# snap-research/MMVID

Measured on AMD Instinct MI355X. Metric: video-tokens/sec training step, 8-frame 128px text-to-video, higher is better.
Workload: dtype bf16

## Files before the change

### mmvid_amd/csrc/common.h

```cpp
#pragma once
#include <hip/hip_runtime.h>
#include <stdint.h>
#include <stdio.h>
#include <stdlib.h>
#include <string.h>

typedef uint16_t bf16_t;
typedef __attribute__((ext_vector_type(8))) __bf16 bf16x8_t;
typedef __attribute__((ext_vector_type(8))) _Float16 f16x8_t;
typedef __attribute__((ext_vector_type(4))) float f32x4;
typedef __attribute__((ext_vector_type(16))) float f32x16;

#define MMVID_OK 0
#define MMVID_ERR_ARG 1
#define MMVID_ERR_HIP 2

extern "C" const char* mmvid_last_error();
void mmvid_set_error(const char* fmt, ...);

#define MMVID_REQUIRE(cond, ...)          \
    do {                                  \
        if (!(cond)) {                    \
            mmvid_set_error(__VA_ARGS__); \
            return MMVID_ERR_ARG;         \
        }                                 \
    } while (0)

#define MMVID_LAUNCH_CHECK(name)                                               \
    do {                                                                       \
        hipError_t e__ = hipGetLastError();                                    \
        if (e__ != hipSuccess) {                                               \
            mmvid_set_error("%s: launch failed: %s", name, hipGetErrorString(e__)); \
            return MMVID_ERR_HIP;                                              \
        }                                                                      \
    } while (0)

typedef __attribute__((ext_vector_type(2))) float f32x2;
typedef __attribute__((ext_vector_type(2))) __bf16 bf16x2_t;
__device__ __forceinline__ float bf2f(bf16_t v) { return __uint_as_float(((uint32_t)v) << 16); }
__device__ __forceinline__ uint32_t pack_bf2(float lo, float hi) {
    const f32x2 v = {lo, hi};
    return __builtin_bit_cast(uint32_t, __builtin_convertvector(v, bf16x2_t));
}
__device__ __forceinline__ bf16_t f2bf(float f) { return (bf16_t)(pack_bf2(f, f) & 0xffffu); }
__device__ __forceinline__ float bf_lo(uint32_t w) { return __uint_as_float(w << 16); }
__device__ __forceinline__ float bf_hi(uint32_t w) { return __uint_as_float(w & 0xffff0000u); }

__device__ __forceinline__ float sigmoidf_(float x) { return 1.0f / (1.0f + __expf(-x)); }

__device__ __forceinline__ float wave_sum(float v) {
#pragma unroll
    for (int o = 32; o > 0; o >>= 1) v += __shfl_xor(v, o, 64);
    return v;
}
__device__ __forceinline__ float wave_max(float v) {
#pragma unroll
    for (int o = 32; o > 0; o >>= 1) v = fmaxf(v, __shfl_xor(v, o, 64));
    return v;
}

template <int CTRL>
__device__ __forceinline__ float dpp_mov(float v) {
    return __builtin_bit_cast(float, __builtin_amdgcn_update_dpp(0, __builtin_bit_cast(int, v), CTRL, 0xf, 0xf, true));
}
__device__ __forceinline__ float wave_sum_fast(float v) {
    v += dpp_mov<0xB1>(v);
    v += dpp_mov<0x4E>(v);
    v += dpp_mov<0x141>(v);
    v += dpp_mov<0x140>(v);
    const uint32_t u = __float_as_uint(v);
    const auto r = __builtin_amdgcn_permlane16_swap(u, u, false, false);
    v = __uint_as_float(r[0]) + __uint_as_float(r[1]);
    const uint32_t w = __float_as_uint(v);
    const auto q = __builtin_amdgcn_permlane32_swap(w, w, false, false);
    return __uint_as_float(q[0]) + __uint_as_float(q[1]);
}
__device__ __forceinline__ float wave_max_fast(float v) {
    v = fmaxf(v, dpp_mov<0xB1>(v));
    v = fmaxf(v, dpp_mov<0x4E>(v));
    v = fmaxf(v, dpp_mov<0x141>(v));
    v = fmaxf(v, dpp_mov<0x140>(v));
    const uint32_t u = __float_as_uint(v);
    const auto r = __builtin_amdgcn_permlane16_swap(u, u, false, false);
    v = fmaxf(__uint_as_float(r[0]), __uint_as_float(r[1]));
    const uint32_t w = __float_as_uint(v);
    const auto q = __builtin_amdgcn_permlane32_swap(w, w, false, false);
    return fmaxf(__uint_as_float(q[0]), __uint_as_float(q[1]));
}

__device__ __forceinline__ void mfma_settle(f32x16& acc) { asm volatile("s_nop 15" : "+v"(acc)); }
__device__ __forceinline__ void mfma_settle(f32x4& acc) { asm volatile("s_nop 15" : "+v"(acc)); }

static inline int cdiv(long a, long b) { return (int)((a + b - 1) / b); }
static inline float* gn_stats_partials(float* area, int N, int C) { return area + (long)N * C * 2; }
enum { MMVID_OPT_GRAPHS = 0, MMVID_OPT_DETERMINISTIC = 1, MMVID_OPT_COUNT = 2 };
int mmvid_option(int which);
int mmvid_slab_reduce(const float* slab, int nslabs, int N, float* out, hipStream_t stream);
unsigned long long* mmvid_fault_counters_dev();
```

### mmvid_amd/csrc/norm.hip

```cpp
#include "../../include/mmvid_hip.h"
#include "common.h"
#include <type_traits>

namespace {

constexpr int LN_MAXV = 4;

__global__ __launch_bounds__(256) void layernorm_fwd_kernel(const float* __restrict__ x, long ldx, long rows, int E,
                                                            const float* __restrict__ w,
                                                            const float* __restrict__ b, float eps,
                                                            bf16_t* __restrict__ y_bf16, float* __restrict__ y_f32,
                                                            long ldy, float* __restrict__ mean_out,
                                                            float* __restrict__ rstd_out) {
    const long half = (rows + 1) >> 1;
    const long r0 = (long)blockIdx.x * 4 + (threadIdx.x >> 6);
    if (r0 >= half) return;
    const long rr[2] = {r0, r0 + half};
    const bool live1 = rr[1] < rows;
    const int lane = threadIdx.x & 63;
    const int nv = E >> 2;
    float4 v[2][LN_MAXV];
    float s[2] = {0.f, 0.f};
#pragma unroll
    for (int k = 0; k < 2; ++k) {
        const float4* xr = reinterpret_cast<const float4*>(x + (k == 0 || live1 ? rr[k] : rr[0]) * ldx);
#pragma unroll
        for (int i = 0; i < LN_MAXV; ++i) {
            const int c = lane + 64 * i;
            v[k][i] = c < nv ? xr[c] : make_float4(0, 0, 0, 0);
        }
    }
#pragma unroll
    for (int k = 0; k < 2; ++k)
#pragma unroll
        for (int i = 0; i < LN_MAXV; ++i) s[k] += (v[k][i].x + v[k][i].y) + (v[k][i].z + v[k][i].w);
    const float mean[2] = {wave_sum_fast(s[0]) / (float)E, wave_sum_fast(s[1]) / (float)E};
    float q[2] = {0.f, 0.f};
#pragma unroll
    for (int k = 0; k < 2; ++k)
#pragma unroll
        for (int i = 0; i < LN_MAXV; ++i) {
            const int c = lane + 64 * i;
            if (c < nv) {
                const float a = v[k][i].x - mean[k], b2 = v[k][i].y - mean[k], c2 = v[k][i].z - mean[k], d = v[k][i].w - mean[k];
                q[k] += (a * a + b2 * b2) + (c2 * c2 + d * d);
            }
        }
    const float rstd[2] = {rsqrtf(wave_sum_fast(q[0]) / (float)E + eps), rsqrtf(wave_sum_fast(q[1]) / (float)E + eps)};
#pragma unroll
    for (int k = 0; k < 2; ++k) {
        if (k == 1 && !live1) break;
        const long r = rr[k];
        if (lane == 0) {
            if (mean_out) mean_out[r] = mean[k];
            if (rstd_out) rstd_out[r] = rstd[k];
        }
#pragma unroll
        for (int i = 0; i < LN_MAXV; ++i) {
            const int c = lane + 64 * i;
            if (c < nv) {
                const float4 w4 = reinterpret_cast<const float4*>(w)[c];
                const float4 b4 = reinterpret_cast<const float4*>(b)[c];
                float4 o;
                o.x = (v[k][i].x - mean[k]) * rstd[k] * w4.x + b4.x;
                o.y = (v[k][i].y - mean[k]) * rstd[k] * w4.y + b4.y;
                o.z = (v[k][i].z - mean[k]) * rstd[k] * w4.z + b4.z;
                o.w = (v[k][i].w - mean[k]) * rstd[k] * w4.w + b4.w;
                if (y_f32) reinterpret_cast<float4*>(y_f32 + r * ldy)[c] = o;
                if (y_bf16) reinterpret_cast<uint2*>(y_bf16 + r * ldy)[c] = make_uint2(pack_bf2(o.x, o.y), pack_bf2(o.z, o.w));
            }
        }
    }
}

template <typename DY>
__global__ __launch_bounds__(256) void layernorm_bwd_kernel(const DY* __restrict__ dy, long lddy,
                                                            const float* __restrict__ x, long ldx,
                                                            const float* __restrict__ mean,
                                                            const float* __restrict__ rstd,
                                                            const float* __restrict__ w, long rows, int E,
                                                            float* __restrict__ dx, long lddx, int add,
                                                            bf16_t* __restrict__ dx_bf16,
                                                            float* __restrict__ dw, float* __restrict__ db,
                                                            float* __restrict__ dx_colsum, float* __restrict__ partial) {
    __shared__ float red[2][4][LN_MAXV * 64 * 4];
    const int lane = threadIdx.x & 63, wave = threadIdx.x >> 6;
    const int nv = E >> 2;
    float4 pw[LN_MAXV], pb[LN_MAXV], pc[LN_MAXV], w4[LN_MAXV];
#pragma unroll
    for (int i = 0; i < LN_MAXV; ++i) {
        pw[i] = pb[i] = pc[i] = make_float4(0, 0, 0, 0);
        const int c = lane + 64 * i;
        w4[i] = (c < nv) ? reinterpret_cast<const float4*>(w)[c] : make_float4(0, 0, 0, 0);
    }
    for (long r = (long)blockIdx.x * 4 + wave; r < rows; r += (long)gridDim.x * 4) {
        const float mu = mean[r], rs = rstd[r];
        float4 g[LN_MAXV], xh[LN_MAXV], prev[LN_MAXV];
        float s1 = 0.f, s2 = 0.f;
#pragma unroll
        for (int i = 0; i < LN_MAXV; ++i) {
            const int c = lane + 64 * i;
            if (c < nv) {
                prev[i] = add ? reinterpret_cast<const float4*>(dx + r * lddx)[c] : make_float4(0.f, 0.f, 0.f, 0.f);
                float4 d4;
                if constexpr (sizeof(DY) == 4) {
                    d4 = reinterpret_cast<const float4*>(dy + r * lddy)[c];
                } else {
                    const uint2 u = reinterpret_cast<const uint2*>(dy + r * lddy)[c];
                    d4 = make_float4(bf_lo(u.x), bf_hi(u.x), bf_lo(u.y), bf_hi(u.y));
                }
                const float4 x4 = reinterpret_cast<const float4*>(x + r * ldx)[c];
                xh[i] = make_float4((x4.x - mu) * rs, (x4.y - mu) * rs, (x4.z - mu) * rs, (x4.w - mu) * rs);
                g[i] = make_float4(d4.x * w4[i].x, d4.y * w4[i].y, d4.z * w4[i].z, d4.w * w4[i].w);
                s1 += (g[i].x + g[i].y) + (g[i].z + g[i].w);
                s2 += (g[i].x * xh[i].x + g[i].y * xh[i].y) + (g[i].z * xh[i].z + g[i].w * xh[i].w);
                pw[i].x += d4.x * xh[i].x, pw[i].y += d4.y * xh[i].y, pw[i].z += d4.z * xh[i].z, pw[i].w += d4.w * xh[i].w;
                pb[i].x += d4.x, pb[i].y += d4.y, pb[i].z += d4.z, pb[i].w += d4.w;
            }
        }
        const float m1 = wave_sum_fast(s1) / (float)E, m2 = wave_sum_fast(s2) / (float)E;
#pragma unroll
        for (int i = 0; i < LN_MAXV; ++i) {
            const int c = lane + 64 * i;
            if (c < nv) {
                float4 o;
                o.x = rs * (g[i].x - m1 - xh[i].x * m2);
                o.y = rs * (g[i].y - m1 - xh[i].y * m2);
                o.z = rs * (g[i].z - m1 - xh[i].z * m2);
                o.w = rs * (g[i].w - m1 - xh[i].w * m2);
                float4* d = reinterpret_cast<float4*>(dx + r * lddx) + c;
                o.x += prev[i].x, o.y += prev[i].y, o.z += prev[i].z, o.w += prev[i].w;
                *d = o;
                pc[i].x += o.x, pc[i].y += o.y, pc[i].z += o.z, pc[i].w += o.w;
                if (dx_bf16)
                    reinterpret_cast<uint2*>(dx_bf16 + r * lddx)[c] = make_uint2(pack_bf2(o.x, o.y), pack_bf2(o.z, o.w));
            }
        }
    }
// ... 395 lines not shown
        }
        const long at = ((long)n * hw + p) * C + c0 + cc * 8;
        if (y_bf16)
            *reinterpret_cast<uint4*>(y_bf16 + at) = make_uint4(pack_bf2(o[0], o[1]), pack_bf2(o[2], o[3]), pack_bf2(o[4], o[5]), pack_bf2(o[6], o[7]));
        if (y_f32) {
            float4* d = reinterpret_cast<float4*>(y_f32 + at);
            d[0] = make_float4(o[0], o[1], o[2], o[3]);
            d[1] = make_float4(o[4], o[5], o[6], o[7]);
        }
    }
}

__global__ __launch_bounds__(256) void groupnorm_finalize_f64_kernel(const float* __restrict__ partial, int nblk, int N, int C,
                                                                     double cnt, float eps, float* __restrict__ mr) {
    const int item = blockIdx.x * 4 + (threadIdx.x >> 6);
    if (item >= N * 32) return;
    const int lane = threadIdx.x & 63;
    const int n = item >> 5, grp = item & 31;
    double sm = 0.0, sq = 0.0;
    for (int k = lane; k < nblk; k += 64) {
        const float2 v = *reinterpret_cast<const float2*>(partial + (((long)n * nblk + k) * 32 + grp) * 2);
        sm += (double)v.x, sq += (double)v.y;
    }
    for (int o = 32; o > 0; o >>= 1) sm += __shfl_xor(sm, o, 64), sq += __shfl_xor(sq, o, 64);
    const double mu = sm / cnt;
    double var = sq / cnt - mu * mu;
    var = var < 0.0 ? 0.0 : var;
    const double rstd = 1.0 / sqrt(var + (double)eps);
    const int cpg = C >> 5;
    if (lane < cpg) *reinterpret_cast<float2*>(mr + ((long)n * C + grp * cpg + lane) * 2) = make_float2((float)mu, (float)rstd);
}

template <bool F16>
__global__ __launch_bounds__(256) void groupnorm_apply_split_kernel(const float* __restrict__ x, long hw, int C,
                                                                    const float* __restrict__ mr, const float* __restrict__ w,
                                                                    const float* __restrict__ b, int swish,
                                                                    bf16_t* __restrict__ planes, long total_chunks) {
    const long t = (long)blockIdx.x * 256 + threadIdx.x;
    if (t >= total_chunks) return;
    const int cchunks = C >> 3;
    const int cc = (int)(t % cchunks);
    const long pix = t / cchunks;
    const int n = (int)(pix / hw);
    float f[8], wv[8], bv[8];
    load8<float>(x + pix * C + cc * 8, f);
    load8<float>(w + cc * 8, wv);
    load8<float>(b + cc * 8, bv);
    const float4* q = reinterpret_cast<const float4*>(mr + ((long)n * C + cc * 8) * 2);
    const float4 q0 = q[0], q1 = q[1], q2 = q[2], q3 = q[3];
    const float mu[8] = {q0.x, q0.z, q1.x, q1.z, q2.x, q2.z, q3.x, q3.z};
    const float rs[8] = {q0.y, q0.w, q1.y, q1.w, q2.y, q2.w, q3.y, q3.w};
    uint32_t h[4], l[4];
    float o[8];
#pragma unroll
    for (int e = 0; e < 8; ++e) {
        float v = ((f[e] - mu[e]) * rs[e]) * wv[e] + bv[e];
        if (swish) v = v * (1.0f / (1.0f + expf(-v)));
        o[e] = v;
    }
    if constexpr (F16) {
#pragma unroll
        for (int e = 0; e < 4; ++e) {
            typedef __attribute__((ext_vector_type(2))) _Float16 h2_t;
            const h2_t p2 = {(_Float16)o[2 * e], (_Float16)o[2 * e + 1]};
            h[e] = __builtin_bit_cast(uint32_t, p2);
        }
        *reinterpret_cast<uint4*>(planes + t * 8) = make_uint4(h[0], h[1], h[2], h[3]);
        return;
    }
#pragma unroll
    for (int e = 0; e < 4; ++e) {
        h[e] = pack_bf2(o[2 * e], o[2 * e + 1]);
        l[e] = pack_bf2(o[2 * e] - bf_lo(h[e]), o[2 * e + 1] - bf_hi(h[e]));
    }
    *reinterpret_cast<uint4*>(planes + t * 8) = make_uint4(h[0], h[1], h[2], h[3]);
    *reinterpret_cast<uint4*>(planes + (total_chunks + t) * 8) = make_uint4(l[0], l[1], l[2], l[3]);
}

}

extern "C" int mmvid_layernorm_fwd(const float* x, int64_t ldx, int64_t rows, int E, const float* w, const float* b,
                                   float eps, void* y_bf16, float* y_f32, int64_t ldy, float* mean, float* rstd,
                                   void* stream) {
    MMVID_REQUIRE(x && w && b && (y_bf16 || y_f32), "layernorm_fwd: null pointer");
    MMVID_REQUIRE(E % 4 == 0 && E <= 64 * 4 * LN_MAXV && ldx % 4 == 0 && ldy % 4 == 0,
                  "layernorm_fwd: E=%d must be a multiple of 4 and <= %d; row strides multiples of 4", E,
                  64 * 4 * LN_MAXV);
    if (rows == 0) return MMVID_OK;
    hipLaunchKernelGGL(layernorm_fwd_kernel, dim3(cdiv((rows + 1) / 2, 4)), dim3(256), 0, (hipStream_t)stream, x, (long)ldx,
                       (long)rows, E, w, b, eps, (bf16_t*)y_bf16, y_f32, (long)ldy, mean, rstd);
    MMVID_LAUNCH_CHECK("layernorm_fwd");
    return MMVID_OK;
}

extern "C" int mmvid_layernorm_bwd_ws(const float* dy, int64_t lddy, const float* x, int64_t ldx, const float* mean,
                                      const float* rstd, const float* w, int64_t rows, int E, float* dx, int64_t lddx,
                                      int add_into_dx, void* dx_bf16, float* dw, float* db, float* dx_colsum,
                                      float* workspace, int64_t workspace_floats, void* stream);
extern "C" int mmvid_layernorm_bwd_ex(const void* dy, int dy_is_bf16, int64_t lddy, const float* x, int64_t ldx, const float* mean,
                                      const float* rstd, const float* w, int64_t rows, int E, float* dx, int64_t lddx,
                                      int add_into_dx, void* dx_bf16, float* dw, float* db, float* dx_colsum,
                                      float* workspace, int64_t workspace_floats, void* stream);

extern "C" int mmvid_layernorm_bwd(const float* dy, int64_t lddy, const float* x, int64_t ldx, const float* mean,
                                   const float* rstd, const float* w, int64_t rows, int E, float* dx, int64_t lddx,
                                   int add_into_dx, void* dx_bf16, float* dw, float* db, float* dx_colsum,
                                   void* stream) {
    return mmvid_layernorm_bwd_ws(dy, lddy, x, ldx, mean, rstd, w, rows, E, dx, lddx, add_into_dx, dx_bf16, dw, db, dx_colsum,
                                  nullptr, 0, stream);
}

extern "C" int mmvid_layernorm_bwd_ws(const float* dy, int64_t lddy, const float* x, int64_t ldx, const float* mean,
                                      const float* rstd, const float* w, int64_t rows, int E, float* dx, int64_t lddx,
                                      int add_into_dx, void* dx_bf16, float* dw, float* db, float* dx_colsum,
                                      float* workspace, int64_t workspace_floats, void* stream) {
    return mmvid_layernorm_bwd_ex(dy, 0, lddy, x, ldx, mean, rstd, w, rows, E, dx, lddx, add_into_dx, dx_bf16, dw, db, dx_colsum,
                                  workspace, workspace_floats, stream);
}

static int layernorm_bwd_impl(const void* dy, int dy_is_bf16, int64_t lddy, const float* x, int64_t ldx, const float* mean,
                              const float* rstd, const float* w, int64_t rows, int E, float* dx, int64_t lddx, int add_into_dx,
                              void* dx_bf16, float* dw, float* db, float* dx_colsum, float* workspace, int64_t workspace_floats,
                              int* blocks_out, void* stream) {
    MMVID_REQUIRE(dy && x && mean && rstd && w && dx, "layernorm_bwd: null pointer");
    MMVID_REQUIRE(E % 4 == 0 && E <= 64 * 4 * LN_MAXV && lddy % 4 == 0 && ldx % 4 == 0 && lddx % 4 == 0,
                  "layernorm_bwd: bad E/strides");
    if (rows == 0) return MMVID_OK;
    int blocks = cdiv(rows, 4);
    const bool any_red = dw || db || dx_colsum;
    float* partial = nullptr;
    if (workspace && any_red) {
        int cap = (int)(workspace_floats / (3 * (int64_t)E));
        if (cap > 2048) cap = 2048;
        if (cap >= 64) {
            if (blocks > cap) blocks = cap;
            partial = workspace;
        }
    }
    MMVID_REQUIRE(partial || !any_red || !mmvid_option(MMVID_OPT_DETERMINISTIC),
                  "layernorm_bwd: deterministic mode refuses the atomic dw / db / dx_colsum sums: pass a workspace of at least 64 * 3 * E "
                  "floats (mmvid_layernorm_bwd_ws / mmvid_layernorm_bwd_ex / mmvid_layernorm_bwd_partial)");
    if (!partial) {
        if (blocks > 512) blocks = 512;
    }
    float* const a_dw = partial ? (dw ? dw : workspace) : dw;
    float* const a_db = partial ? (db ? db : workspace) : db;
    float* const a_cs = partial ? (dx_colsum ? dx_colsum : nullptr) : dx_colsum;
    if (E == 768 || E == 512) {
#define MMVID_LN_FAST(DYT, NVI)                                                                                                            \
    hipLaunchKernelGGL((layernorm_bwd_fast_kernel<DYT, NVI>), dim3(blocks), dim3(256), 0, (hipStream_t)stream, (const DYT*)dy, (long)lddy, x, \
                       (long)ldx, mean, rstd, w, (long)rows, dx, (long)lddx, add_into_dx, (bf16_t*)dx_bf16, a_dw, a_db, a_cs, partial)
        if (dy_is_bf16) {
            if (E == 768) MMVID_LN_FAST(bf16_t, 3); else MMVID_LN_FAST(bf16_t, 2);
        } else {
            if (E == 768) MMVID_LN_FAST(float, 3); else MMVID_LN_FAST(float, 2);
        }
#undef MMVID_LN_FAST
    } else if (dy_is_bf16)
        hipLaunchKernelGGL(layernorm_bwd_kernel<bf16_t>, dim3(blocks), dim3(256), 0, (hipStream_t)stream, (const bf16_t*)dy, (long)lddy, x,
                           (long)ldx, mean, rstd, w, (long)rows, E, dx, (long)lddx, add_into_dx, (bf16_t*)dx_bf16,
                           partial ? (dw ? dw : workspace) : dw, partial ? (db ? db : workspace) : db,
                           partial ? (dx_colsum ? dx_colsum : nullptr) : dx_colsum, partial);
    else
        hipLaunchKernelGGL(layernorm_bwd_kernel<float>, dim3(blocks), dim3(256), 0, (hipStream_t)stream, (const float*)dy, (long)lddy, x,
                           (long)ldx, mean, rstd, w, (long)rows, E, dx, (long)lddx, add_into_dx, (bf16_t*)dx_bf16,
                           partial ? (dw ? dw : workspace) : dw, partial ? (db ? db : workspace) : db,
                           partial ? (dx_colsum ? dx_colsum : nullptr) : dx_colsum, partial);
    if (blocks_out) {
        MMVID_REQUIRE(partial || !any_red, "layernorm_bwd_partial: needs a workspace of at least 64 * 3 * E floats");
        *blocks_out = blocks;
    } else if (partial) {
        hipLaunchKernelGGL(layernorm_bwd_reduce_kernel, dim3(cdiv(E, 32), 3), dim3(1024), 0, (hipStream_t)stream, partial, blocks, E,
                           dw, db, dx_colsum);
// ... 127 lines not shown
```

### mmvid_amd/csrc/optim.hip

```cpp
#include "../../include/mmvid_hip.h"
#include "common.h"

namespace {

__global__ __launch_bounds__(256) void grad_sqnorm_kernel(const float* __restrict__ g, long n,
                                                          float* __restrict__ out) {
    float a = 0.f;
    const long stride = (long)gridDim.x * 256 * 4;
    for (long i = ((long)blockIdx.x * 256 + threadIdx.x) * 4; i < n; i += stride) {
        if (i + 3 < n) {
            const float4 v = *reinterpret_cast<const float4*>(g + i);
            a += (v.x * v.x + v.y * v.y) + (v.z * v.z + v.w * v.w);
        } else {
            for (long k = i; k < n; ++k) a += g[k] * g[k];
        }
    }
    a = wave_sum(a);
    __shared__ float sh[4];
    if ((threadIdx.x & 63) == 0) sh[threadIdx.x >> 6] = a;
    __syncthreads();
    if (threadIdx.x == 0) unsafeAtomicAdd(out, (sh[0] + sh[1]) + (sh[2] + sh[3]));
}

struct AdamArgs {
    float lr, beta1, beta2, eps, weight_decay, bc1, bc2_sqrt, max_norm, grad_scale;
};
struct LazyRows {
    const unsigned char* flags;
    long lo, hi;
    int rowlen;
};
__device__ __forceinline__ bool lazy_skip(const LazyRows& z, long i) {
    return z.flags && i >= z.lo && i < z.hi && z.flags[(i - z.lo) / z.rowlen] == 0;
}

__global__ __launch_bounds__(256) void adam_kernel(float* __restrict__ p, const float* __restrict__ g,
                                                   float* __restrict__ m, float* __restrict__ v,
                                                   bf16_t* __restrict__ shadow, long n, AdamArgs a,
                                                   const float* __restrict__ sqnorm,
                                                   const float* __restrict__ step_dev,
                                                   const float* __restrict__ lr_dev, LazyRows z) {
    if (lr_dev) a.lr = *lr_dev;
    if (step_dev) {
        const float t = *step_dev;
        a.bc1 = 1.0f - powf(a.beta1, t);
        a.bc2_sqrt = sqrtf(1.0f - powf(a.beta2, t));
    }
    float coef = a.grad_scale;
    if (sqnorm && a.max_norm > 0.f) {
        const float c = a.max_norm / (sqrtf(*sqnorm) * a.grad_scale + 1e-6f);
        coef *= c < 1.f ? c : 1.f;
    }
    const float step = a.lr / a.bc1;
    const long stride = (long)gridDim.x * 256 * 4;
    for (long i = ((long)blockIdx.x * 256 + threadIdx.x) * 4; i < n; i += stride) {
        if (lazy_skip(z, i)) continue;
        if (i + 3 < n) {
            float4 pp = *reinterpret_cast<float4*>(p + i);
            const float4 gg = *reinterpret_cast<const float4*>(g + i);
            float4 mm = *reinterpret_cast<float4*>(m + i), vv = *reinterpret_cast<float4*>(v + i);
            float pe[4] = {pp.x, pp.y, pp.z, pp.w}, ge[4] = {gg.x, gg.y, gg.z, gg.w};
            float me[4] = {mm.x, mm.y, mm.z, mm.w}, ve[4] = {vv.x, vv.y, vv.z, vv.w};
#pragma unroll
            for (int e = 0; e < 4; ++e) {
                float gr = ge[e] * coef + a.weight_decay * pe[e];
                me[e] = a.beta1 * me[e] + (1.f - a.beta1) * gr;
                ve[e] = a.beta2 * ve[e] + (1.f - a.beta2) * gr * gr;
                pe[e] -= step * me[e] / (sqrtf(ve[e]) / a.bc2_sqrt + a.eps);
            }
            *reinterpret_cast<float4*>(p + i) = make_float4(pe[0], pe[1], pe[2], pe[3]);
            *reinterpret_cast<float4*>(m + i) = make_float4(me[0], me[1], me[2], me[3]);
            *reinterpret_cast<float4*>(v + i) = make_float4(ve[0], ve[1], ve[2], ve[3]);
            if (shadow) *reinterpret_cast<uint2*>(shadow + i) = make_uint2(pack_bf2(pe[0], pe[1]), pack_bf2(pe[2], pe[3]));
        } else {
            for (long k = i; k < n; ++k) {
                float gr = g[k] * coef + a.weight_decay * p[k];
                float mk = a.beta1 * m[k] + (1.f - a.beta1) * gr;
                float vk = a.beta2 * v[k] + (1.f - a.beta2) * gr * gr;
                float pk = p[k] - step * mk / (sqrtf(vk) / a.bc2_sqrt + a.eps);
                p[k] = pk, m[k] = mk, v[k] = vk;
                if (shadow) shadow[k] = f2bf(pk);
            }
        }
    }
}

__global__ __launch_bounds__(256) void cast_bf16_kernel(const float* __restrict__ x, bf16_t* __restrict__ y, long n) {
    const long stride = (long)gridDim.x * 256 * 4;
    for (long i = ((long)blockIdx.x * 256 + threadIdx.x) * 4; i < n; i += stride) {
        if (i + 3 < n) {
            const float4 v = *reinterpret_cast<const float4*>(x + i);
            *reinterpret_cast<uint2*>(y + i) = make_uint2(pack_bf2(v.x, v.y), pack_bf2(v.z, v.w));
        } else {
            for (long k = i; k < n; ++k) y[k] = f2bf(x[k]);
        }
    }
}

static int grid_for(long n) {
    long b = (n + 1023) / 1024;
    if (b > 2048) b = 2048;
    if (b < 1) b = 1;
    return (int)b;
}

}

extern "C" int mmvid_grad_sqnorm(const float* g, int64_t n, float* out_accum, void* stream) {
    MMVID_REQUIRE(g && out_accum && n >= 0, "grad_sqnorm: bad arguments");
    MMVID_REQUIRE(((uintptr_t)g & 15) == 0, "grad_sqnorm: buffer must be 16-byte aligned");
    if (n == 0) return MMVID_OK;
    hipLaunchKernelGGL(grad_sqnorm_kernel, dim3(grid_for(n)), dim3(256), 0, (hipStream_t)stream, g, (long)n, out_accum);
    MMVID_LAUNCH_CHECK("grad_sqnorm");
    return MMVID_OK;
}

__global__ __launch_bounds__(256) void grad_sqnorm_partial_kernel(const float* __restrict__ g, long n, float* __restrict__ part,
                                                                  LazyRows z) {
    float a = 0.f;
    const long stride = (long)gridDim.x * 256 * 4;
    for (long i = ((long)blockIdx.x * 256 + threadIdx.x) * 4; i < n; i += stride) {
        if (lazy_skip(z, i)) continue;
        if (i + 3 < n) {
            const float4 v = *reinterpret_cast<const float4*>(g + i);
            a += (v.x * v.x + v.y * v.y) + (v.z * v.z + v.w * v.w);
        } else {
            for (long k = i; k < n; ++k) a += g[k] * g[k];
        }
    }
    a = wave_sum(a);
    __shared__ float sh[4];
    if ((threadIdx.x & 63) == 0) sh[threadIdx.x >> 6] = a;
    __syncthreads();
    if (threadIdx.x == 0) part[blockIdx.x] = (sh[0] + sh[1]) + (sh[2] + sh[3]);
}
__global__ __launch_bounds__(256) void sum_partials_kernel(const float* __restrict__ part, int nb, float* __restrict__ out) {
    __shared__ float sh[256];
    float a = 0.f;
    for (int i = threadIdx.x; i < nb; i += 256) a += part[i];
    sh[threadIdx.x] = a;
    __syncthreads();
    for (int o = 128; o > 0; o >>= 1) {
        if ((int)threadIdx.x < o) sh[threadIdx.x] += sh[threadIdx.x + o];
        __syncthreads();
    }
    if (threadIdx.x == 0) out[0] += sh[0];
}

static int make_lazy(LazyRows& z, const uint8_t* flags, int64_t lo, int64_t rows, int rowlen, int64_t n) {
    z.flags = nullptr, z.lo = z.hi = 0, z.rowlen = 1;
    if (!flags) return MMVID_OK;
    MMVID_REQUIRE(lo >= 0 && rows >= 0 && rowlen > 0 && rowlen % 4 == 0 && lo % 4 == 0 && lo + rows * rowlen <= n,
                  "lazy rows: the table [%lld, +%lld x %d) must lie inside the buffer and be 4-element aligned", (long long)lo,
                  (long long)rows, rowlen);
    z.flags = flags, z.lo = lo, z.hi = lo + rows * rowlen, z.rowlen = rowlen;
    return MMVID_OK;
}

extern "C" int mmvid_grad_sqnorm_det(const float* g, int64_t n, float* partials, float* out_accum, void* stream) {
    return mmvid_grad_sqnorm_rows(g, n, partials, out_accum, nullptr, 0, 0, 0, stream);
}

extern "C" int mmvid_grad_sqnorm_rows(const float* g, int64_t n, float* partials, float* out_accum, const uint8_t* row_flags,
                                      int64_t table_lo, int64_t table_rows, int rowlen, void* stream) {
    MMVID_REQUIRE(g && partials && out_accum && n >= 0, "grad_sqnorm_det: bad arguments");
    MMVID_REQUIRE(((uintptr_t)g & 15) == 0, "grad_sqnorm_det: buffer must be 16-byte aligned");
    if (n == 0) return MMVID_OK;
    LazyRows z;
    if (int rc = make_lazy(z, row_flags, table_lo, table_rows, rowlen, n)) return rc;
    const int nb = grid_for(n);
    hipLaunchKernelGGL(grad_sqnorm_partial_kernel, dim3(nb), dim3(256), 0, (hipStream_t)stream, g, (long)n, partials, z);
    hipLaunchKernelGGL(sum_partials_kernel, dim3(1), dim3(256), 0, (hipStream_t)stream, partials, nb, out_accum);
    MMVID_LAUNCH_CHECK("grad_sqnorm_det");
    return MMVID_OK;
}

extern "C" int mmvid_adam_step_lr(float* p, const float* g, float* m, float* v, void* shadow_bf16, int64_t n, float lr,
                                  const float* lr_dev, float beta1, float beta2, float eps, float weight_decay, int step,
                                  const float* step_dev, float max_norm, const float* sqnorm, float grad_scale, void* stream);

extern "C" int mmvid_adam_step(float* p, const float* g, float* m, float* v, void* shadow_bf16, int64_t n, float lr,
                               float beta1, float beta2, float eps, float weight_decay, int step,
                               const float* step_dev, float max_norm, const float* sqnorm, float grad_scale,
                               void* stream) {
    return mmvid_adam_step_lr(p, g, m, v, shadow_bf16, n, lr, nullptr, beta1, beta2, eps, weight_decay, step, step_dev, max_norm,
                              sqnorm, grad_scale, stream);
}

extern "C" int mmvid_adam_step_lr(float* p, const float* g, float* m, float* v, void* shadow_bf16, int64_t n, float lr,
                                  const float* lr_dev, float beta1, float beta2, float eps, float weight_decay, int step,
                                  const float* step_dev, float max_norm, const float* sqnorm, float grad_scale, void* stream) {
    return mmvid_adam_step_rows(p, g, m, v, shadow_bf16, n, lr, lr_dev, beta1, beta2, eps, weight_decay, step, step_dev, max_norm,
                                sqnorm, grad_scale, nullptr, 0, 0, 0, stream);
}

extern "C" int mmvid_adam_step_rows(float* p, const float* g, float* m, float* v, void* shadow_bf16, int64_t n, float lr,
                                    const float* lr_dev, float beta1, float beta2, float eps, float weight_decay, int step,
                                    const float* step_dev, float max_norm, const float* sqnorm, float grad_scale,
                                    const uint8_t* row_flags, int64_t table_lo, int64_t table_rows, int rowlen, void* stream) {
    MMVID_REQUIRE(p && g && m && v && n >= 0 && (step >= 1 || step_dev), "adam_step: bad arguments");
    MMVID_REQUIRE(!row_flags || weight_decay == 0.f, "adam_step: lazy rows are exact only without weight decay");
    LazyRows z;
    if (int rc = make_lazy(z, row_flags, table_lo, table_rows, rowlen, n)) return rc;
    MMVID_REQUIRE((((uintptr_t)p | (uintptr_t)g | (uintptr_t)m | (uintptr_t)v) & 15) == 0 && ((uintptr_t)shadow_bf16 & 7) == 0,
                  "adam_step: buffers must be 16-byte aligned");
    if (n == 0) return MMVID_OK;
    AdamArgs a;
    a.lr = lr, a.beta1 = beta1, a.beta2 = beta2, a.eps = eps, a.weight_decay = weight_decay;
    a.bc1 = 1.0f - powf(beta1, (float)(step >= 1 ? step : 1));
    a.bc2_sqrt = sqrtf(1.0f - powf(beta2, (float)(step >= 1 ? step : 1)));
    a.max_norm = max_norm, a.grad_scale = grad_scale;
    hipLaunchKernelGGL(adam_kernel, dim3(grid_for(n)), dim3(256), 0, (hipStream_t)stream, p, g, m, v, (bf16_t*)shadow_bf16,
                       (long)n, a, sqnorm, step_dev, lr_dev, z);
    MMVID_LAUNCH_CHECK("adam_step");
    return MMVID_OK;
}

extern "C" int mmvid_cast_f32_to_bf16(const float* x, void* y, int64_t n, void* stream) {
    MMVID_REQUIRE(x && y && n >= 0, "cast_f32_to_bf16: bad arguments");
    MMVID_REQUIRE(((uintptr_t)x & 15) == 0 && ((uintptr_t)y & 7) == 0, "cast_f32_to_bf16: alignment");
    if (n == 0) return MMVID_OK;
    hipLaunchKernelGGL(cast_bf16_kernel, dim3(grid_for(n)), dim3(256), 0, (hipStream_t)stream, x, (bf16_t*)y, (long)n);
    MMVID_LAUNCH_CHECK("cast_f32_to_bf16");
    return MMVID_OK;
}
```

### mmvid_amd/csrc/tower.hip

```cpp
#include "../../include/mmvid_hip.h"
#include "common.h"
#include <vector>

#include "graphs.h"

namespace {

inline int64_t align256(int64_t x) { return (x + 255) & ~(int64_t)255; }
constexpr int kMaxSplitK = 16;
constexpr int kLnBwdBlocks = 512;

struct Dims {
    int B, L, E, H, F, layers;
    int64_t M;
};
Dims dims_of(const mmvid_tower_cfg_t& c) {
    Dims d;
    d.B = c.B, d.L = c.L, d.E = c.E, d.H = c.H, d.F = c.F, d.layers = c.layers;
    d.M = (int64_t)c.B * c.L;
    return d;
}

struct SavedLayer {
    int64_t x_in, x_mid, mean1, rstd1, mean2, rstd2, h1, qkv, o, lse2, h2, pre, act, k_gpj, k_dpre, k_gout, k_dqkv, k_ln1, k_ln2, total;
// ... 53 lines not shown

#define TRY(call)                   \
    do {                            \
        int rc__ = (call);          \
        if (rc__ != 0) return rc__; \
    } while (0)

int check_cfg(const mmvid_tower_cfg_t* c) {
    MMVID_REQUIRE(c, "tower: null config");
    MMVID_REQUIRE(c->B > 0 && c->L > 0 && c->layers > 0, "tower: bad B/L/layers");
    MMVID_REQUIRE(c->E == c->H * 64 && c->E % 8 == 0 && c->F % 8 == 0 && c->E <= 1024,
                  "tower: need E == 64*H <= 1024 and F %% 8 == 0 (E=%d H=%d F=%d)", c->E, c->H, c->F);
    return 0;
}

int linear_fwd(int64_t M, int N, int K, const void* X, const void* W, const float* bias, const float* residual,
               void* save_pre, int act, float* out_f32, void* out_bf16, void* st) {
    return mmvid_gemm_bf16(0, 0, (int)M, N, K, X, K, W, K, 1, 0, 0, 0, 1, 1.0f, bias, residual, N, nullptr, save_pre, N,
                           act, 0, out_f32, out_bf16, N, nullptr, st);
}
int linear_dx(int64_t M, int N, int K, const void* dY, const void* W, const void* dact_pre, float* out_f32,
              void* out_bf16, void* st, float* out_colsum = nullptr, void* det_ws = nullptr, int64_t det_bytes = 0) {
    if (out_colsum && det_ws)
        return mmvid_gemm_bf16_det(0, 1, (int)M, K, N, dY, N, W, K, 1, 0, 0, 0, 1, 1.0f, nullptr, nullptr, 0, dact_pre, nullptr, K,
                                   0, 0, out_f32, out_bf16, K, out_colsum, det_ws, det_bytes, st);
    return mmvid_gemm_bf16(0, 1, (int)M, K, N, dY, N, W, K, 1, 0, 0, 0, 1, 1.0f, nullptr, nullptr, 0, dact_pre, nullptr, K,
                           0, 0, out_f32, out_bf16, K, out_colsum, st);
}
int linear_dw(int64_t M, int N, int K, const void* dY, const void* X, float* dW, float* db, float* ws, void* st) {
    if (dW) {
        const int sk = mmvid_gemm_dw_pick_splitk(M, N, K);
        TRY(mmvid_gemm_bf16_dw(M, N, K, dY, N, X, K, sk, ws, dW, 1, st));
    }
    if (db) TRY(mmvid_colsum_bf16(dY, N, M, N, db, st));
    return 0;
}

}

extern "C" int mmvid_tower_workspace(const mmvid_tower_cfg_t* cfg, int64_t* saved_bytes, int64_t* scratch_bytes) {
    TRY(check_cfg(cfg));
    const Dims d = dims_of(*cfg);
    if (saved_bytes) *saved_bytes = saved_layout(d).total * d.layers;
    if (scratch_bytes) *scratch_bytes = scratch_layout(d).total;
    return MMVID_OK;
}

static int tower_forward_enqueue(const mmvid_tower_cfg_t* cfg, const mmvid_tower_layer_t* layers, const float* x_in,
                                 float* x_out, void* saved, void* scratch, void* stream, void* kv_cache = nullptr,
                                 int kv_lmax = 0);
static int tower_backward_enqueue(const mmvid_tower_cfg_t* cfg, const mmvid_tower_layer_t* layers, float* g,
                                  void* saved, void* scratch, void* stream);

static uint64_t tower_key(uint64_t seed, const mmvid_tower_cfg_t* cfg, const mmvid_tower_layer_t* layers, const void* a,
                          const void* b, const void* c, const void* d, const void* stream) {
    uint64_t k = mmvid_hash_bytes(cfg, sizeof(*cfg), 0xcbf29ce484222325ull ^ seed);
    k = mmvid_hash_bytes(layers, sizeof(mmvid_tower_layer_t) * (size_t)cfg->layers, k);
    return mmvid_hash_ptr(stream, mmvid_hash_ptr(d, mmvid_hash_ptr(c, mmvid_hash_ptr(b, mmvid_hash_ptr(a, k)))));
}

extern "C" int mmvid_tower_forward(const mmvid_tower_cfg_t* cfg, const mmvid_tower_layer_t* layers,
                                   const float* x_in, float* x_out, void* saved, void* scratch, void* stream) {
    TRY(check_cfg(cfg));
    MMVID_REQUIRE(layers && x_in && x_out && scratch, "tower_forward: null pointer");
    const uint64_t key = tower_key(2, cfg, layers, x_in, x_out, saved, scratch, stream);
    return mmvid_run_cached(key, (hipStream_t)stream, [=](hipStream_t s) {
        return tower_forward_enqueue(cfg, layers, x_in, x_out, saved, scratch, (void*)s);
    });
}

static int tower_forward_enqueue(const mmvid_tower_cfg_t* cfg, const mmvid_tower_layer_t* layers, const float* x_in,
                                 float* x_out, void* saved, void* scratch, void* stream, void* kv_cache, int kv_lmax) {
    const Dims d = dims_of(*cfg);
    const SavedLayer sl = saved_layout(d);
    const Scratch sc = scratch_layout(d);
    char* scr = (char*)scratch;
    const float scale = 0.125f;
    const float* x = x_in;
    for (int i = 0; i < d.layers; ++i) {
        const mmvid_tower_layer_t& ly = layers[i];
        char* sv = saved ? (char*)saved + (int64_t)i * sl.total : scr + sc.infer;
        float* xin_s = (float*)(sv + sl.x_in);
        float* xmid = (float*)(sv + sl.x_mid);
        if (saved && i == 0) {
            if (hipMemcpyAsync(xin_s, x_in, d.M * d.E * 4, hipMemcpyDeviceToDevice, (hipStream_t)stream) != hipSuccess) {
                mmvid_set_error("tower_forward: memcpy failed");
                return MMVID_ERR_HIP;
            }
            x = xin_s;
        }
        float* xnext;
        if (i == d.layers - 1)
            xnext = x_out;
        else if (saved)
            xnext = (float*)((char*)saved + (int64_t)(i + 1) * sl.total + sl.x_in);
        else
            xnext = x_out;
        TRY(mmvid_layernorm_fwd(x, d.E, d.M, d.E, ly.ln1_w, ly.ln1_b, cfg->ln_eps, sv + sl.h1, nullptr, d.E,
                                (float*)(sv + sl.mean1), (float*)(sv + sl.rstd1), stream));
        TRY(linear_fwd(d.M, 3 * d.E, d.E, sv + sl.h1, ly.in_w, ly.in_b, nullptr, nullptr, 0, nullptr, sv + sl.qkv, stream));
        if (kv_cache)
            TRY(mmvid_kv_store(sv + sl.qkv, 3 * d.E, d.B, d.L, d.E, nullptr, 0, kv_lmax,
                               (char*)kv_cache + (int64_t)i * d.B * kv_lmax * 2 * d.E * 2, stream));
        TRY(mmvid_attention_fwd(sv + sl.qkv, 3 * d.E, d.B, d.L, d.H, d.E, scale, cfg->mask_mode, cfg->r0, cfg->c0, cfg->r1,
                                cfg->c1, sv + sl.o, d.E, (float*)(sv + sl.lse2), stream));
        TRY(linear_fwd(d.M, d.E, d.E, sv + sl.o, ly.out_w, ly.out_b, x, nullptr, 0, xmid, nullptr, stream));
        TRY(mmvid_layernorm_fwd(xmid, d.E, d.M, d.E, ly.ln2_w, ly.ln2_b, cfg->ln_eps, sv + sl.h2, nullptr, d.E,
                                (float*)(sv + sl.mean2), (float*)(sv + sl.rstd2), stream));
        TRY(linear_fwd(d.M, d.F, d.E, sv + sl.h2, ly.fc_w, ly.fc_b, nullptr, saved ? sv + sl.pre : nullptr, 1, nullptr,
                       sv + sl.act, stream));
        TRY(linear_fwd(d.M, d.E, d.F, sv + sl.act, ly.pj_w, ly.pj_b, xmid, nullptr, 0, xnext, nullptr, stream));
        x = xnext;
    }
    return MMVID_OK;
}

extern "C" int mmvid_tower_backward(const mmvid_tower_cfg_t* cfg, const mmvid_tower_layer_t* layers, float* g,
                                    void* saved, void* scratch, void* stream) {
    TRY(check_cfg(cfg));
    MMVID_REQUIRE(layers && g && saved && scratch, "tower_backward: null pointer");
    const uint64_t key = tower_key(mmvid_option(MMVID_OPT_DETERMINISTIC) ? 5 : 3, cfg, layers, g, saved, scratch, nullptr, stream);
    return mmvid_run_cached(key, (hipStream_t)stream, [=](hipStream_t s) {
        return tower_backward_enqueue(cfg, layers, g, saved, scratch, (void*)s);
    });
}

static int tower_backward_enqueue(const mmvid_tower_cfg_t* cfg, const mmvid_tower_layer_t* layers, float* g, void* saved,
                                  void* scratch, void* stream) {
    const Dims d = dims_of(*cfg);
    const SavedLayer sl = saved_layout(d);
    const Scratch sc = scratch_layout(d);
    char* scr = (char*)scratch;
    char* keep = (char*)saved;
    struct { int64_t g_pj, d_pre, g_out, dqkv, total; } kl = {sl.k_gpj, sl.k_dpre, sl.k_gout, sl.k_dqkv, sl.total};
    const float scale = 0.125f;
    void* d_h = scr + sc.d_h;
    float* ws = (float*)(scr + sc.splitk_ws);
    void* det_ws = nullptr;
    const int64_t det_bytes = det_slab_bytes(d);
    if (mmvid_option(MMVID_OPT_DETERMINISTIC)) {
        MMVID_REQUIRE(det_bytes <= sc.total - sc.infer, "tower_backward: the deterministic slabs do not fit the scratch arena");
        det_ws = scr + sc.infer;
    }
    const int64_t ln_ws_floats = (int64_t)kLnBwdBlocks * 3 * d.E;
    std::vector<mmvid_ln_reduce_t> ln_items;
    int ln_blocks = 0;
    for (int i = d.layers - 1; i >= 0; --i) {
        const mmvid_tower_layer_t& ly = layers[i];
        const char* sv = (const char*)saved + (int64_t)i * sl.total;
        char* kp = keep + (int64_t)i * kl.total;
        void* g_pj = kp + kl.g_pj;
        if (i == d.layers - 1) {
            TRY(mmvid_cast_f32_to_bf16(g, g_pj, d.M * d.E, stream));
            if (ly.g_pj_b && det_ws) TRY(mmvid_colsum_bf16_det(g_pj, d.E, d.M, d.E, ly.g_pj_b, det_ws, det_bytes, stream));
            if (ly.g_pj_b && !det_ws) TRY(mmvid_colsum_bf16(g_pj, d.E, d.M, d.E, ly.g_pj_b, stream));
        }
        TRY(linear_dx(d.M, d.E, d.F, g_pj, ly.pj_w, sv + sl.pre, nullptr, kp + kl.d_pre, stream, ly.g_fc_b, det_ws, det_bytes));
        TRY(linear_dx(d.M, d.F, d.E, kp + kl.d_pre, ly.fc_w, nullptr, nullptr, d_h, stream));
        {
            mmvid_ln_reduce_t r = {(const float*)(kp + sl.k_ln2), ly.g_ln2_w, ly.g_ln2_b, ly.g_out_b};
            int nb = 0;
            TRY(mmvid_layernorm_bwd_partial(d_h, 1, d.E, (const float*)(sv + sl.x_mid), d.E, (const float*)(sv + sl.mean2),
                                            (const float*)(sv + sl.rstd2), ly.ln2_w, d.M, d.E, g, d.E, 1, kp + kl.g_out, r.dw != nullptr,
                                            r.db != nullptr, r.dx_colsum != nullptr, (float*)(kp + sl.k_ln2), ln_ws_floats, &nb, stream));
            if (r.dw || r.db || r.dx_colsum) ln_items.push_back(r), ln_blocks = nb;
        }
        TRY(linear_dx(d.M, d.E, d.E, kp + kl.g_out, ly.out_w, nullptr, nullptr, scr + sc.d_o, stream));
        if (det_ws)
            TRY(mmvid_attention_bwd_bias_det(sv + sl.qkv, 3 * d.E, sv + sl.o, d.E, scr + sc.d_o, d.E, (const float*)(sv + sl.lse2),
                                             (float*)(scr + sc.delta), d.B, d.L, d.H, d.E, scale, cfg->mask_mode, cfg->r0, cfg->c0,
                                             cfg->r1, cfg->c1, kp + kl.dqkv, 3 * d.E, ly.g_in_b, det_ws, det_bytes, stream));
        else
            TRY(mmvid_attention_bwd_bias(sv + sl.qkv, 3 * d.E, sv + sl.o, d.E, scr + sc.d_o, d.E, (const float*)(sv + sl.lse2),
                                         (float*)(scr + sc.delta), d.B, d.L, d.H, d.E, scale, cfg->mask_mode, cfg->r0, cfg->c0,
                                         cfg->r1, cfg->c1, kp + kl.dqkv, 3 * d.E, ly.g_in_b, stream));
        TRY(linear_dx(d.M, 3 * d.E, d.E, kp + kl.dqkv, ly.in_w, nullptr, nullptr, d_h, stream));
        {
            mmvid_ln_reduce_t r = {(const float*)(kp + sl.k_ln1), ly.g_ln1_w, ly.g_ln1_b, i > 0 ? layers[i - 1].g_pj_b : nullptr};
            int nb = 0;
            TRY(mmvid_layernorm_bwd_partial(d_h, 1, d.E, (const float*)(sv + sl.x_in), d.E, (const float*)(sv + sl.mean1),
                                            (const float*)(sv + sl.rstd1), ly.ln1_w, d.M, d.E, g, d.E, 1,
                                            i > 0 ? (void*)(keep + (int64_t)(i - 1) * kl.total + kl.g_pj) : nullptr, r.dw != nullptr,
// ... 84 lines not shown
```

Measured before the change: 216,900.

## Fuse tower input save into layernorm and restructure Adam lazy-row sweep

The first layer's input copy is now written by the layernorm forward kernel while it already holds the row in registers, instead of a separate device-to-device memcpy. The Adam kernel is also restructured. It sweeps the dense part of the buffer outside the lazy embedding table with two float4 groups per thread, then visits only flagged table rows using a wave ballot, instead of checking a per-element skip predicate across the whole buffer. The launch grid is also recomputed from the dense size and row count. The Adam arithmetic is rewritten with explicit fma and contraction disabled, which may change rounding slightly.

After: 217,700 (median of 6 runs). Within noise of the previous version (+0.4%).

```diff
diff --git a/mmvid_amd/csrc/common.h b/mmvid_amd/csrc/common.h
--- a/mmvid_amd/csrc/common.h
+++ b/mmvid_amd/csrc/common.h
@@ -95,5 +95,7 @@
 static inline float* gn_stats_partials(float* area, int N, int C) { return area + (long)N * C * 2; }
 enum { MMVID_OPT_GRAPHS = 0, MMVID_OPT_DETERMINISTIC = 1, MMVID_OPT_COUNT = 2 };
 int mmvid_option(int which);
+int layernorm_fwd_launch(const float* x, int64_t ldx, int64_t rows, int E, const float* w, const float* b, float eps, void* y_bf16,
+                         float* y_f32, int64_t ldy, float* mean, float* rstd, float* x_copy, int64_t ldc, void* stream);
 int mmvid_slab_reduce(const float* slab, int nslabs, int N, float* out, hipStream_t stream);
 unsigned long long* mmvid_fault_counters_dev();
diff --git a/mmvid_amd/csrc/norm.hip b/mmvid_amd/csrc/norm.hip
--- a/mmvid_amd/csrc/norm.hip
+++ b/mmvid_amd/csrc/norm.hip
@@ -11,7 +11,7 @@
                                                             const float* __restrict__ b, float eps,
                                                             bf16_t* __restrict__ y_bf16, float* __restrict__ y_f32,
                                                             long ldy, float* __restrict__ mean_out,
-                                                            float* __restrict__ rstd_out) {
+                                                            float* __restrict__ rstd_out, float* __restrict__ x_copy, long ldc) {
     const long half = (rows + 1) >> 1;
     const long r0 = (long)blockIdx.x * 4 + (threadIdx.x >> 6);
     if (r0 >= half) return;
@@ -54,6 +54,13 @@
         if (lane == 0) {
             if (mean_out) mean_out[r] = mean[k];
             if (rstd_out) rstd_out[r] = rstd[k];
+        }
+        if (x_copy) {
+#pragma unroll
+            for (int i = 0; i < LN_MAXV; ++i) {
+                const int c = lane + 64 * i;
+                if (c < nv) reinterpret_cast<float4*>(x_copy + r * ldc)[c] = v[k][i];
+            }
         }
 #pragma unroll
         for (int i = 0; i < LN_MAXV; ++i) {
@@ -615,13 +622,18 @@
 extern "C" int mmvid_layernorm_fwd(const float* x, int64_t ldx, int64_t rows, int E, const float* w, const float* b,
                                    float eps, void* y_bf16, float* y_f32, int64_t ldy, float* mean, float* rstd,
                                    void* stream) {
+    return layernorm_fwd_launch(x, ldx, rows, E, w, b, eps, y_bf16, y_f32, ldy, mean, rstd, nullptr, 0, stream);
+}
+
+int layernorm_fwd_launch(const float* x, int64_t ldx, int64_t rows, int E, const float* w, const float* b, float eps, void* y_bf16,
+                         float* y_f32, int64_t ldy, float* mean, float* rstd, float* x_copy, int64_t ldc, void* stream) {
     MMVID_REQUIRE(x && w && b && (y_bf16 || y_f32), "layernorm_fwd: null pointer");
-    MMVID_REQUIRE(E % 4 == 0 && E <= 64 * 4 * LN_MAXV && ldx % 4 == 0 && ldy % 4 == 0,
+    MMVID_REQUIRE(E % 4 == 0 && E <= 64 * 4 * LN_MAXV && ldx % 4 == 0 && ldy % 4 == 0 && (!x_copy || (ldc % 4 == 0 && ldc >= E)),
                   "layernorm_fwd: E=%d must be a multiple of 4 and <= %d; row strides multiples of 4", E,
                   64 * 4 * LN_MAXV);
     if (rows == 0) return MMVID_OK;
     hipLaunchKernelGGL(layernorm_fwd_kernel, dim3(cdiv((rows + 1) / 2, 4)), dim3(256), 0, (hipStream_t)stream, x, (long)ldx,
-                       (long)rows, E, w, b, eps, (bf16_t*)y_bf16, y_f32, (long)ldy, mean, rstd);
+                       (long)rows, E, w, b, eps, (bf16_t*)y_bf16, y_f32, (long)ldy, mean, rstd, x_copy, (long)ldc);
     MMVID_LAUNCH_CHECK("layernorm_fwd");
     return MMVID_OK;
 }
diff --git a/mmvid_amd/csrc/optim.hip b/mmvid_amd/csrc/optim.hip
--- a/mmvid_amd/csrc/optim.hip
+++ b/mmvid_amd/csrc/optim.hip
@@ -29,9 +29,52 @@
     const unsigned char* flags;
     long lo, hi;
     int rowlen;
+    long rows;
 };
 __device__ __forceinline__ bool lazy_skip(const LazyRows& z, long i) {
     return z.flags && i >= z.lo && i < z.hi && z.flags[(i - z.lo) / z.rowlen] == 0;
+}
+
+__device__ __forceinline__ void adam_elem(float& p, float g, float& m, float& v, const AdamArgs& a, float coef, float step) {
+#pragma clang fp contract(off)
+    const float gr = __builtin_fmaf(g, coef, a.weight_decay * p);
+    m = __builtin_fmaf(a.beta1, m, (1.f - a.beta1) * gr);
+    v = __builtin_fmaf(a.beta2, v, ((1.f - a.beta2) * gr) * gr);
+    p = p - (step * m) / (sqrtf(v) / a.bc2_sqrt + a.eps);
+}
+
+struct Adam4 {
+    float4 p, g, m, v;
+};
+__device__ __forceinline__ void adam_load4(Adam4& r, const float* p, const float* g, const float* m, const float* v, long i) {
+    r.p = *reinterpret_cast<const float4*>(p + i), r.g = *reinterpret_cast<const float4*>(g + i);
+    r.m = *reinterpret_cast<const float4*>(m + i), r.v = *reinterpret_cast<const float4*>(v + i);
+}
+__device__ __forceinline__ void adam_update4(const Adam4& r, float* p, float* m, float* v, bf16_t* shadow, long i, const AdamArgs& a,
+                                             float coef, float step) {
+    float pe[4] = {r.p.x, r.p.y, r.p.z, r.p.w}, ge[4] = {r.g.x, r.g.y, r.g.z, r.g.w};
+    float me[4] = {r.m.x, r.m.y, r.m.z, r.m.w}, ve[4] = {r.v.x, r.v.y, r.v.z, r.v.w};
+#pragma unroll
+    for (int e = 0; e < 4; ++e) adam_elem(pe[e], ge[e], me[e], ve[e], a, coef, step);
+    *reinterpret_cast<float4*>(p + i) = make_float4(pe[0], pe[1], pe[2], pe[3]);
+    *reinterpret_cast<float4*>(m + i) = make_float4(me[0], me[1], me[2], me[3]);
+    *reinterpret_cast<float4*>(v + i) = make_float4(ve[0], ve[1], ve[2], ve[3]);
+    if (shadow) *reinterpret_cast<uint2*>(shadow + i) = make_uint2(pack_bf2(pe[0], pe[1]), pack_bf2(pe[2], pe[3]));
+}
+__device__ __forceinline__ void adam_group_or_tail(float* p, const float* g, float* m, float* v, bf16_t* shadow, long i, long n,
+                                                   const AdamArgs& a, float coef, float step) {
+    if (i + 3 < n) {
+        Adam4 r;
+        adam_load4(r, p, g, m, v, i);
+        adam_update4(r, p, m, v, shadow, i, a, coef, step);
+    } else {
+        for (long k = i; k < n; ++k) {
+            float pk = p[k], mk = m[k], vk = v[k];
+            adam_elem(pk, g[k], mk, vk, a, coef, step);
+            p[k] = pk, m[k] = mk, v[k] = vk;
+            if (shadow) shadow[k] = f2bf(pk);
+        }
+    }
 }
 
 __global__ __launch_bounds__(256) void adam_kernel(float* __restrict__ p, const float* __restrict__ g,
@@ -52,34 +95,41 @@
         coef *= c < 1.f ? c : 1.f;
     }
     const float step = a.lr / a.bc1;
-    const long stride = (long)gridDim.x * 256 * 4;
-    for (long i = ((long)blockIdx.x * 256 + threadIdx.x) * 4; i < n; i += stride) {
-        if (lazy_skip(z, i)) continue;
-        if (i + 3 < n) {
-            float4 pp = *reinterpret_cast<float4*>(p + i);
-            const float4 gg = *reinterpret_cast<const float4*>(g + i);
-            float4 mm = *reinterpret_cast<float4*>(m + i), vv = *reinterpret_cast<float4*>(v + i);
-            float pe[4] = {pp.x, pp.y, pp.z, pp.w}, ge[4] = {gg.x, gg.y, gg.z, gg.w};
-            float me[4] = {mm.x, mm.y, mm.z, mm.w}, ve[4] = {vv.x, vv.y, vv.z, vv.w};
-#pragma unroll
-            for (int e = 0; e < 4; ++e) {
-                float gr = ge[e] * coef + a.weight_decay * pe[e];
-                me[e] = a.beta1 * me[e] + (1.f - a.beta1) * gr;
-                ve[e] = a.beta2 * ve[e] + (1.f - a.beta2) * gr * gr;
-                pe[e] -= step * me[e] / (sqrtf(ve[e]) / a.bc2_sqrt + a.eps);
-            }
-            *reinterpret_cast<float4*>(p + i) = make_float4(pe[0], pe[1], pe[2], pe[3]);
-            *reinterpret_cast<float4*>(m + i) = make_float4(me[0], me[1], me[2], me[3]);
-            *reinterpret_cast<float4*>(v + i) = make_float4(ve[0], ve[1], ve[2], ve[3]);
-            if (shadow) *reinterpret_cast<uint2*>(shadow + i) = make_uint2(pack_bf2(pe[0], pe[1]), pack_bf2(pe[2], pe[3]));
-        } else {
-            for (long k = i; k < n; ++k) {
-                float gr = g[k] * coef + a.weight_decay * p[k];
-                float mk = a.beta1 * m[k] + (1.f - a.beta1) * gr;
-                float vk = a.beta2 * v[k] + (1.f - a.beta2) * gr * gr;
-                float pk = p[k] - step * mk / (sqrtf(vk) / a.bc2_sqrt + a.eps);
-                p[k] = pk, m[k] = mk, v[k] = vk;
-                if (shadow) shadow[k] = f2bf(pk);
+    const long gap = z.hi - z.lo;
+    const long nd = n - gap;
+    const long stride = (long)gridDim.x * 2048;
+    for (long j0 = (long)blockIdx.x * 2048 + threadIdx.x * 4; j0 < nd; j0 += stride) {
+        const long j1 = j0 + 1024;
+        const long i0 = j0 < z.lo ? j0 : j0 + gap, i1 = j1 < z.lo ? j1 : j1 + gap;
+        if (j1 + 3 < nd) {
+            Adam4 r0, r1;
+            adam_load4(r0, p, g, m, v, i0);
+            adam_load4(r1, p, g, m, v, i1);
+            adam_update4(r0, p, m, v, shadow, i0, a, coef, step);
+            adam_update4(r1, p, m, v, shadow, i1, a, coef, step);
+        } else {
+            adam_group_or_tail(p, g, m, v, shadow, i0, n, a, coef, step);
+            if (j1 < nd) adam_group_or_tail(p, g, m, v, shadow, i1, n, a, coef, step);
+        }
+    }
+    if (!z.flags) return;
+    const int lane = threadIdx.x & 63;
+    const long wave = (long)blockIdx.x * 4 + (threadIdx.x >> 6), nwaves = (long)gridDim.x * 4;
+    const int nv = z.rowlen >> 2;
+    for (long r0 = wave; r0 < z.rows; r0 += 64 * nwaves) {
+        const long mine = r0 + lane * nwaves;
+        unsigned long long todo = __ballot(mine < z.rows && z.flags[mine] != 0);
+        while (todo) {
+            const int l = __ffsll(todo) - 1;
+            todo &= todo - 1;
+            const long base = z.lo + (r0 + l * nwaves) * z.rowlen;
+            for (int c = lane; c < nv; c += 128) {
+                const long i0 = base + 4L * c, i1 = i0 + 256;
+                Adam4 r0v, r1v;
+                adam_load4(r0v, p, g, m, v, i0);
+                if (c + 64 < nv) adam_load4(r1v, p, g, m, v, i1);
+                adam_update4(r0v, p, m, v, shadow, i0, a, coef, step);
+                if (c + 64 < nv) adam_update4(r1v, p, m, v, shadow, i1, a, coef, step);
             }
         }
     }
@@ -148,12 +198,12 @@
 }
 
 static int make_lazy(LazyRows& z, const uint8_t* flags, int64_t lo, int64_t rows, int rowlen, int64_t n) {
-    z.flags = nullptr, z.lo = z.hi = 0, z.rowlen = 1;
+    z.flags = nullptr, z.lo = z.hi = 0, z.rowlen = 1, z.rows = 0;
     if (!flags) return MMVID_OK;
     MMVID_REQUIRE(lo >= 0 && rows >= 0 && rowlen > 0 && rowlen % 4 == 0 && lo % 4 == 0 && lo + rows * rowlen <= n,
                   "lazy rows: the table [%lld, +%lld x %d) must lie inside the buffer and be 4-element aligned", (long long)lo,
                   (long long)rows, rowlen);
-    z.flags = flags, z.lo = lo, z.hi = lo + rows * rowlen, z.rowlen = rowlen;
+    z.flags = flags, z.lo = lo, z.hi = lo + rows * rowlen, z.rowlen = rowlen, z.rows = rows;
     return MMVID_OK;
 }
 
@@ -210,7 +260,10 @@
     a.bc1 = 1.0f - powf(beta1, (float)(step >= 1 ? step : 1));
     a.bc2_sqrt = sqrtf(1.0f - powf(beta2, (float)(step >= 1 ? step : 1)));
     a.max_norm = max_norm, a.grad_scale = grad_scale;
-    hipLaunchKernelGGL(adam_kernel, dim3(grid_for(n)), dim3(256), 0, (hipStream_t)stream, p, g, m, v, (bf16_t*)shadow_bf16,
+    long blocks = (n - (z.hi - z.lo) + 2047) / 2048;
+    if (blocks < (z.rows + 3) / 4) blocks = (z.rows + 3) / 4;
+    blocks = blocks > 1536 ? 1536 : blocks < 1 ? 1 : blocks;
+    hipLaunchKernelGGL(adam_kernel, dim3((int)blocks), dim3(256), 0, (hipStream_t)stream, p, g, m, v, (bf16_t*)shadow_bf16,
                        (long)n, a, sqnorm, step_dev, lr_dev, z);
     MMVID_LAUNCH_CHECK("adam_step");
     return MMVID_OK;
diff --git a/mmvid_amd/csrc/tower.hip b/mmvid_amd/csrc/tower.hip
--- a/mmvid_amd/csrc/tower.hip
+++ b/mmvid_amd/csrc/tower.hip
@@ -159,13 +159,7 @@
         char* sv = saved ? (char*)saved + (int64_t)i * sl.total : scr + sc.infer;
         float* xin_s = (float*)(sv + sl.x_in);
         float* xmid = (float*)(sv + sl.x_mid);
-        if (saved && i == 0) {
-            if (hipMemcpyAsync(xin_s, x_in, d.M * d.E * 4, hipMemcpyDeviceToDevice, (hipStream_t)stream) != hipSuccess) {
-                mmvid_set_error("tower_forward: memcpy failed");
-                return MMVID_ERR_HIP;
-            }
-            x = xin_s;
-        }
+        const bool save_x = saved && i == 0 && xin_s != x_in;
         float* xnext;
         if (i == d.layers - 1)
             xnext = x_out;
@@ -173,8 +167,9 @@
             xnext = (float*)((char*)saved + (int64_t)(i + 1) * sl.total + sl.x_in);
         else
             xnext = x_out;
-        TRY(mmvid_layernorm_fwd(x, d.E, d.M, d.E, ly.ln1_w, ly.ln1_b, cfg->ln_eps, sv + sl.h1, nullptr, d.E,
-                                (float*)(sv + sl.mean1), (float*)(sv + sl.rstd1), stream));
+        TRY(layernorm_fwd_launch(x, d.E, d.M, d.E, ly.ln1_w, ly.ln1_b, cfg->ln_eps, sv + sl.h1, nullptr, d.E, (float*)(sv + sl.mean1),
+                                 (float*)(sv + sl.rstd1), save_x ? xin_s : nullptr, d.E, stream));
+        if (save_x) x = xin_s;
         TRY(linear_fwd(d.M, 3 * d.E, d.E, sv + sl.h1, ly.in_w, ly.in_b, nullptr, nullptr, 0, nullptr, sv + sl.qkv, stream));
         if (kv_cache)
             TRY(mmvid_kv_store(sv + sl.qkv, 3 * d.E, d.B, d.L, d.E, nullptr, 0, kv_lmax,
```
